# scrose/SVDSolver

Measured on NVIDIA B200. Metric: bidiag_reduction_gflops, higher is better.
Workload: dtype f64,f32

## Files before the change

svdsolver_b200/csrc/capi.cu:

```cuda
#include <algorithm>
#include <new>
#include "common.cuh"

using namespace svdb200;

namespace svdb200 {
template <typename T, bool kTrans> int launch_panel_public(Ctx* c, T* a, size_t lda, int m, int b, T* V, T* V2, cudaStream_t stream);
namespace {

__device__ __forceinline__ unsigned long long splitmix64(unsigned long long x) {
    x += 0x9E3779B97F4A7C15ull;
    x = (x ^ (x >> 30)) * 0xBF58476D1CE4E5B9ull;
    x = (x ^ (x >> 27)) * 0x94D049BB133111EBull;
    return x ^ (x >> 31);
}
template <typename T>
__global__ void fill_uniform_kernel(T* __restrict__ a, size_t count, unsigned long long seed, double lo, double hi) {
    size_t i = (size_t)blockIdx.x * blockDim.x + threadIdx.x;
    size_t stride = (size_t)gridDim.x * blockDim.x;
    const double span = __dsub_rn(hi, lo);
    for (; i < count; i += stride) {
        double u = __dmul_rn((double)(splitmix64(seed + i) >> 11), 1.0 / 9007199254740992.0);
        a[i] = (T)__dadd_rn(lo, __dmul_rn(span, u));
    }
// ... 235 lines not shown
        Ctx* s = c->pool[i % K];
        inherit_settings(c, s);
        T* ai = a + i * n * n;
        T* d = reinterpret_cast<T*>(s->d);
        T* e = reinterpret_cast<T*>(s->e);
        const long long before = s->launches;
        s->overlap_safe = (concurrent && K > 1) ? 1 : 0;
        const int st1 = stage1_panel_order<T>(s, ai, n, band);
        s->overlap_safe = 0;
        if (st1 != 0) { c->last_error = s->last_error; return st1; }
        SVDB_TRY(stage2_chase<T>(s, ai, n, band, d, e));
        SVDB_TRY(bidiag_qr<T>(s, d, e, n, sigma + i * n));
        c->launches += s->launches - before;
    }
    for (int i = 0; i < K; ++i) {
        SVDB_CHECK(c, cudaEventRecord(c->pool[i]->lev[0], c->pool[i]->stream));
        SVDB_CHECK(c, cudaStreamWaitEvent(c->stream, c->pool[i]->lev[0], 0));
    }
    return 0;
}
template <typename T>
int batched_chain(Ctx* c, T* a, size_t count, size_t n, size_t band, int what, T* d, T* e, T* sigma) {
    if (count == 0) return 0;
    if (!(n <= 1024 && band <= 64 && c->cluster_ok >= 8 && n >= 2)) return SVDB200_E_CAPACITY;
    return batched_small<T>(c, a, count, n, band, sigma, what, d, e);
}
template int batched_chain<float>(Ctx*, float*, size_t, size_t, size_t, int, float*, float*, float*);
template int batched_chain<double>(Ctx*, double*, size_t, size_t, size_t, int, double*, double*, double*);
template int batched_svdvals<float>(Ctx*, float*, size_t, size_t, size_t, float*);
template int batched_svdvals<double>(Ctx*, double*, size_t, size_t, size_t, double*);

constexpr size_t kOverlapMaxN = 4096;

static void release_s2(Ctx* c) {
    for (int l = 0; l < Ctx::kLanes; ++l) {
        if (c->s1ctx[l]) { svdb200_destroy(reinterpret_cast<svdb200_handle>(c->s1ctx[l])); c->s1ctx[l] = nullptr; }
        if (l > 0 && c->s2_prog[l]) cudaFree(c->s2_prog[l]);
        c->s2_prog[l] = nullptr;
        if (c->s2_stream[l]) { cudaStreamDestroy(c->s2_stream[l]); c->s2_stream[l] = nullptr; }
    }
    for (auto& e : c->s2ev) if (e) { cudaEventDestroy(e); e = nullptr; }
    c->s2_ready = 0;
}

static int ensure_s2_impl(Ctx* c) {
    for (int l = 0; l < Ctx::kLanes; ++l) {
        SVDB_CHECK(c, cudaStreamCreateWithFlags(&c->s2_stream[l], cudaStreamNonBlocking));
        if (l == 0) c->s2_prog[l] = c->prog;
        else SVDB_CHECK(c, cudaMalloc(&c->s2_prog[l], sizeof(int) * (c->max_n + 8)));
        svdb200_handle h = nullptr;
        int st = svdb200_create(&h, c->device, c->max_n, c->band, c->dtype);
        if (st != 0) return st;
        c->s1ctx[l] = reinterpret_cast<Ctx*>(h);
    }
    for (auto& e : c->s2ev) SVDB_CHECK(c, cudaEventCreateWithFlags(&e, cudaEventDisableTiming));
    return 0;
}

static int ensure_s2(Ctx* c) {
    if (c->s2_ready) return 0;
    const int st = ensure_s2_impl(c);
    if (st != 0) { release_s2(c); return st; }
    c->s2_ready = 1;
    return 0;
}

static int lanes_for(Ctx* c, size_t n, size_t band) {
    const size_t ctas = n / band / 2 + 2;
    const size_t cap = (size_t)c->num_sms - 8;
    return ((size_t)Ctx::kLanes * ctas <= cap) ? Ctx::kLanes : 1;
}

template <typename T>
static int run_stage2_on_lane(Ctx* c, int lane, T* a, size_t n, size_t band, T* d, T* e) {
    cudaStream_t s0 = c->stream;
    int* p0 = c->prog;
    c->stream = c->s2_stream[lane];
    c->prog = c->s2_prog[lane];
    const int st = stage2_chase<T>(c, a, n, band, d, e);
    c->stream = s0;
    c->prog = p0;
    return st;
}

static int drain_into(Ctx* c, cudaStream_t into) {
    for (int l = 0; l < Ctx::kLanes; ++l) {
        SVDB_CHECK(c, cudaEventRecord(c->s2ev[4 + l], c->s2_stream[l]));
        SVDB_CHECK(c, cudaStreamWaitEvent(into, c->s2ev[4 + l], 0));
        SVDB_CHECK(c, cudaEventRecord(c->s1ctx[l]->lev[0], c->s1ctx[l]->stream));
        SVDB_CHECK(c, cudaStreamWaitEvent(into, c->s1ctx[l]->lev[0], 0));
    }
    return 0;
}

template <typename T>
static int pipeline_one(Ctx* c, size_t i, T* a_dev, const T* a_host, size_t n, size_t band, int order, T* d, T* e, cudaStream_t* lane_out,
                        int k) {
    const bool overlap = order == SVDB200_ORDER_PANEL && n <= kOverlapMaxN && !c->profile;
    const int nl = overlap ? lanes_for(c, n, band) : 1;
    if (!overlap || nl == 1) {
        SVDB_TRY(drain_into(c, c->stream));
        if (a_host) SVDB_CHECK(c, cudaMemcpyAsync(a_dev, a_host, sizeof(T) * n * n, cudaMemcpyHostToDevice, c->stream));
        SVDB_TRY(order == SVDB200_ORDER_PANEL ? stage1_panel_order<T>(c, a_dev, n, band) : stage1_tile_order<T>(c, a_dev, n, band));
        if (i < c->band_capture.size() && c->band_capture[i])
            SVDB_CHECK(c, cudaMemcpyAsync(c->band_capture[i], a_dev, sizeof(T) * n * n, cudaMemcpyDeviceToDevice, c->stream));
        SVDB_TRY(stage2_chase<T>(c, a_dev, n, band, d, e));
        SVDB_CHECK(c, cudaEventRecord(c->s2ev[1], c->stream));
        for (int l = 0; l < Ctx::kLanes; ++l) {
            SVDB_CHECK(c, cudaStreamWaitEvent(c->s2_stream[l], c->s2ev[1], 0));
            SVDB_CHECK(c, cudaStreamWaitEvent(c->s1ctx[l]->stream, c->s2ev[1], 0));
        }
        *lane_out = c->stream;
        return 0;
    }
    Ctx* s = c->s1ctx[k];
    inherit_settings(c, s);
    if (a_host) SVDB_CHECK(c, cudaMemcpyAsync(a_dev, a_host, sizeof(T) * n * n, cudaMemcpyHostToDevice, s->stream));
    s->overlap_safe = 1;
    int st = stage1_panel_order<T>(s, a_dev, n, band);
    s->overlap_safe = 0;
    c->launches += s->launches; s->launches = 0;
    if (st != 0) { c->last_error = s->last_error; return st; }
    if (i < c->band_capture.size() && c->band_capture[i])
        SVDB_CHECK(c, cudaMemcpyAsync(c->band_capture[i], a_dev, sizeof(T) * n * n, cudaMemcpyDeviceToDevice, s->stream));
    SVDB_CHECK(c, cudaEventRecord(s->lev[0], s->stream));
    SVDB_CHECK(c, cudaStreamWaitEvent(c->s2_stream[k], s->lev[0], 0));
    SVDB_TRY(run_stage2_on_lane<T>(c, k, a_dev, n, band, d, e));
    *lane_out = c->s2_stream[k];
    return 0;
}

struct ListPlan { std::vector<size_t> order; std::vector<int> chain; };
static ListPlan plan_list(int lanes, size_t count, const size_t* n) {
    ListPlan pl;
    const int L = lanes < 1 ? 1 : lanes;
    pl.order.reserve(count); pl.chain.reserve(count);
    if (L == 1 || count <= (size_t)L) {
        for (size_t i = 0; i < count; ++i) { pl.order.push_back(i); pl.chain.push_back((int)(i % (size_t)L)); }
        return pl;
    }
    std::vector<size_t> idx(count);
    for (size_t i = 0; i < count; ++i) idx[i] = i;
    std::stable_sort(idx.begin(), idx.end(), [&](size_t x, size_t y) { return n[x] > n[y]; });
    std::vector<std::vector<size_t>> items(L);
    std::vector<size_t> load(L, 0);
    for (size_t i : idx) {
        int best = 0;
        for (int l = 1; l < L; ++l) if (load[l] < load[best]) best = l;
        items[best].push_back(i);
        load[best] += n[i];
    }
    for (auto& v : items) std::stable_sort(v.begin(), v.end(), [&](size_t x, size_t y) { return n[x] != n[y] ? n[x] < n[y] : x < y; });
    for (size_t t = 0; pl.order.size() < count; ++t)
        for (int l = 0; l < L; ++l)
            if (t < items[l].size()) { pl.order.push_back(items[l][t]); pl.chain.push_back(l); }
    return pl;
}

template <typename T>
int bidiagonalize_many_dev(Ctx* c, size_t count, T* const* a, const size_t* n, size_t band, int order, T* const* d, T* const* e) {
    if (count == 0) return 0;
    SVDB_TRY(ensure_s2(c));
    cudaStream_t s0 = c->stream;
    SVDB_CHECK(c, cudaEventRecord(c->s2ev[0], s0));
    for (int l = 0; l < Ctx::kLanes; ++l) {
        SVDB_CHECK(c, cudaStreamWaitEvent(c->s2_stream[l], c->s2ev[0], 0));
        SVDB_CHECK(c, cudaStreamWaitEvent(c->s1ctx[l]->stream, c->s2ev[0], 0));
    }
    const ListPlan pl = plan_list(Ctx::kLanes, count, n);
    for (size_t j = 0; j < count; ++j) {
        const size_t i = pl.order[j];
        cudaStream_t lane;
        SVDB_TRY(pipeline_one<T>(c, i, a[i], (const T*)nullptr, n[i], band, order, d ? d[i] : nullptr, e ? e[i] : nullptr, &lane, pl.chain[j]));
    }
    const int sj = drain_into(c, s0);
    c->band_capture.clear();
    return sj;
}
template int bidiagonalize_many_dev<float>(Ctx*, size_t, float* const*, const size_t*, size_t, int, float* const*, float* const*);
template int bidiagonalize_many_dev<double>(Ctx*, size_t, double* const*, const size_t*, size_t, int, double* const*, double* const*);

static bool is_pageable(const void* p) {
    if (!p) return false;
    cudaPointerAttributes at{};
    if (cudaPointerGetAttributes(&at, p) != cudaSuccess) { cudaGetLastError(); return true; }
    return at.type == cudaMemoryTypeUnregistered;
}

template <typename T>
int bidiagonalize_many_host(Ctx* c, size_t count, T* const* a, const size_t* n, size_t band, int order, T* const* d, T* const* e) {
    if (count == 0) return 0;
    SVDB_TRY(ensure_s2(c));
    constexpr int NB = 2 * Ctx::kLanes;
    if (!c->a_dev) SVDB_CHECK(c, cudaMalloc(&c->a_dev, c->esz * c->max_n * c->max_n));
    c->a_stage[0] = c->a_dev;
    for (int k = 1; k < NB; ++k)
        if (!c->a_stage[k]) SVDB_CHECK(c, cudaMalloc(&c->a_stage[k], c->esz * c->max_n * c->max_n));
    if (!c->de2) SVDB_CHECK(c, cudaMalloc(&c->de2, c->esz * 2 * NB * (c->max_n + 8)));
    cudaStream_t s0 = c->stream;
    SVDB_CHECK(c, cudaEventRecord(c->s2ev[0], s0));
    for (int l = 0; l < Ctx::kLanes; ++l) {
        SVDB_CHECK(c, cudaStreamWaitEvent(c->s2_stream[l], c->s2ev[0], 0));
        SVDB_CHECK(c, cudaStreamWaitEvent(c->s1ctx[l]->stream, c->s2ev[0], 0));
    }
    struct EvSet {
        cudaEvent_t ev[NB] = {};
        ~EvSet() { for (auto& x : ev) if (x) cudaEventDestroy(x); }
    } evs;
    cudaEvent_t* ev_free = evs.ev;
    for (auto& ev : evs.ev) SVDB_CHECK(c, cudaEventCreateWithFlags(&ev, cudaEventDisableTiming));
    struct Result { T *a, *d, *e; size_t n; cudaStream_t lane; bool live; } res[NB] = {};
    auto copy_back = [&](int k) -> int {
        Result& r = res[k];
        if (!r.live) return 0;
        r.live = false;
        T* buf = reinterpret_cast<T*>(c->a_stage[k]);
        T* dd = reinterpret_cast<T*>(c->de2) + (size_t)2 * k * (c->max_n + 8);
        T* ee = dd + (c->max_n + 8);
        SVDB_CHECK(c, cudaMemcpyAsync(r.a, buf, sizeof(T) * r.n * r.n, cudaMemcpyDeviceToHost, r.lane));
        if (r.d) SVDB_CHECK(c, cudaMemcpyAsync(r.d, dd, sizeof(T) * r.n, cudaMemcpyDeviceToHost, r.lane));
        if (r.e) SVDB_CHECK(c, cudaMemcpyAsync(r.e, ee, sizeof(T) * (r.n - 1), cudaMemcpyDeviceToHost, r.lane));
        SVDB_CHECK(c, cudaEventRecord(ev_free[k], r.lane));
        return 0;
    };
    int st = 0;
    const ListPlan pl = plan_list(Ctx::kLanes, count, n);
    size_t per_chain[Ctx::kLanes] = {};
    bool used[NB] = {};
    for (size_t j = 0; j < count && st == 0; ++j) {
        const size_t i = pl.order[j];
        const int ch = pl.chain[j];
        const int k = ch + Ctx::kLanes * (int)(per_chain[ch]++ % 2);
        const size_t ni = n[i];
        T* buf = reinterpret_cast<T*>(c->a_stage[k]);
        T* dd = reinterpret_cast<T*>(c->de2) + (size_t)2 * k * (c->max_n + 8);
        T* ee = dd + (c->max_n + 8);
        if ((st = copy_back(k)) != 0) break;
// ... 178 lines not shown
    SVDB_CREATE_CHECK(cudaMalloc(&c->s, es * band * band));
    SVDB_CREATE_CHECK(cudaMalloc(&c->tau, es * band));
    SVDB_CREATE_CHECK(cudaMalloc(&c->red, es * 2 * (kMaxPanelCtas + 1) * (2 * band + 8)));
    SVDB_CREATE_CHECK(cudaMemset(c->red, 0, es * 2 * (kMaxPanelCtas + 1) * (2 * band + 8)));
    SVDB_CREATE_CHECK(cudaMalloc(&c->red2, 512 * 1024));
    SVDB_CREATE_CHECK(cudaMemset(c->red2, 0, 512 * 1024));
    SVDB_CREATE_CHECK(cudaMalloc(&c->chol_ws, 1 << 20));
    SVDB_CREATE_CHECK(cudaMemset(c->chol_ws, 0, 1 << 20));
    SVDB_CREATE_CHECK(cudaMalloc(&c->bar, 64));
    SVDB_CREATE_CHECK(cudaMemset(c->bar, 0, 64));
    SVDB_CREATE_CHECK(cudaMalloc(&c->prog, sizeof(int) * (max_n + 8)));
    SVDB_CREATE_CHECK(cudaMalloc(&c->d, es * (max_n + 8)));
    SVDB_CREATE_CHECK(cudaMalloc(&c->e, es * (max_n + 8)));
    SVDB_CREATE_CHECK(cudaMalloc(&c->sigma, es * (max_n + 8)));
    SVDB_CREATE_CHECK(cudaMalloc(&c->qr_info, 64));
    SVDB_CREATE_CHECK(cudaMemset(c->qr_info, 0, 64));
    SVDB_CREATE_CHECK(cudaMalloc(&c->tileq, es * (max_n / band + 2) * 4 * band * band));
    SVDB_CREATE_CHECK(cudaMalloc(&c->tilestate, es * (4 * band * band + 64)));
#undef SVDB_CREATE_CHECK
    *out = reinterpret_cast<svdb200_handle>(c);
    return 0;
}

int svdb200_destroy(svdb200_handle h) {
    if (!h) return SVDB200_E_ARG;
    Ctx* c = reinterpret_cast<Ctx*>(h);
    cudaSetDevice(c->device);
    if (c->own_stream) cudaStreamSynchronize(c->own_stream);
    for (auto& ph : c->pool) if (ph) svdb200_destroy(reinterpret_cast<svdb200_handle>(ph));
    c->pool.clear();
    void* ptrs[] = {c->a_dev, c->v, c->v2, c->vb, c->v2b, c->w, c->wpart, c->s, c->tau, c->red, c->red2, c->chol_ws, c->bar, c->prog,
                    c->d, c->e, c->sigma, c->qr_info, c->tileq, c->tilestate, c->tcsplit, c->bis_ws, c->batch_prog, c->batch_ws, c->de2};
    for (int k = 1; k < 2 * Ctx::kLanes; ++k) if (c->a_stage[k]) cudaFree(c->a_stage[k]);
    for (int l = 0; l < Ctx::kLanes; ++l) if (c->s1ctx[l]) svdb200_destroy(reinterpret_cast<svdb200_handle>(c->s1ctx[l]));
    for (int l = 1; l < Ctx::kLanes; ++l) if (c->s2_prog[l]) cudaFree(c->s2_prog[l]);
    for (void* p : ptrs) if (p) cudaFree(p);
    for (auto& e : c->ev) if (e) cudaEventDestroy(e);
    for (auto& e : c->pev) if (e) cudaEventDestroy(e);
    for (auto& e : c->lev) if (e) cudaEventDestroy(e);
    for (auto& e : c->s2ev) if (e) cudaEventDestroy(e);
    for (auto& st2 : c->s2_stream) if (st2) cudaStreamDestroy(st2);
    if (c->aux_stream) cudaStreamDestroy(c->aux_stream);
    if (c->own_stream) cudaStreamDestroy(c->own_stream);
    delete c;
    return 0;
}

int svdb200_set_stream(svdb200_handle h, void* stream) {
    if (!h) return SVDB200_E_ARG;
    Ctx* c = reinterpret_cast<Ctx*>(h);
    c->stream = stream ? reinterpret_cast<cudaStream_t>(stream) : c->own_stream;
    return 0;
}

int svdb200_synchronize(svdb200_handle h) {
    if (!h) return SVDB200_E_ARG;
    Ctx* c = reinterpret_cast<Ctx*>(h);
    SVDB_CHECK(c, cudaStreamSynchronize(c->stream));
    return 0;
}

#define SVDB_ENTER(T)                                    \
    Ctx* c = reinterpret_cast<Ctx*>(h);                  \
    if (!c) return SVDB200_E_ARG;                        \
    if (c->dtype != dtype_of<T>()) return SVDB200_E_ARG; \
    SVDB_CHECK(c, cudaSetDevice(c->device));

#define SVDB_DEFINE_TYPED(T, S)                                                                                          \
// ... 308 lines not shown
```

svdsolver_b200/csrc/common.cuh:

```cuda
#pragma once
#include <cuda_runtime.h>
#include <cstddef>
#include <cstdint>
#include <cstdio>
#include <cstring>
#include <string>
#include <vector>
#include "../../include/svdb200.h"

namespace svdb200 {

constexpr int kMaxBand = 128;
constexpr int kMaxPanelCtas = 148;
constexpr int kLookaheadReserve = 20;

struct Settings {
    int stage2_complete = 0;
    int qr_method = 0;
    size_t qr_auto_limit = 1024;
    int use_tc05 = 1;
    long long tc05_min_elems = 8LL << 20;
    int panel_blk = 1;
    int panel_chol = 1;
    double chol_guard = 1e-3;
};

struct Ctx {
    int device = 0;
    int dtype = SVDB200_F64;
    size_t max_n = 0, band = 0, esz = 8;
    int num_sms = 148;
    cudaStream_t own_stream = nullptr, stream = nullptr;
    void* a_dev = nullptr;
    void* v = nullptr;
    void* v2 = nullptr;
    void* vb = nullptr; void* v2b = nullptr;
    cudaStream_t aux_stream = nullptr;
    cudaEvent_t lev[4] = {};
    void* w = nullptr;
    void* wpart = nullptr;
    size_t wpart_elems = 0;
    void* s = nullptr;
    void* tau = nullptr;
    unsigned panel_epoch = 0;
    void* red = nullptr;
    void* red2 = nullptr;
    unsigned int* bar = nullptr;
    int* prog = nullptr;
    void* d = nullptr; void* e = nullptr; void* sigma = nullptr;
    long long* qr_info = nullptr;
    void* tileq = nullptr;
    void* tilestate = nullptr;
    long long launches = 0;
    cudaEvent_t ev[8] = {};
    double ms_stage1 = 0, ms_stage2 = 0, ms_qr = 0, ms_h2d = 0, ms_d2h = 0;
    std::string last_error;
    int coop_supported = 0;
    int cluster_ok = 16;
    int profile = 0;
    double prof_ms[SVDB200_PROFILE_CLASSES] = {};
    double prof_work[SVDB200_PROFILE_CLASSES] = {};
    long long prof_launches[SVDB200_PROFILE_CLASSES] = {};
    cudaEvent_t pev[2] = {};
    std::vector<Ctx*> pool;
    size_t pool_n = 0, pool_band = 0;
    void* tcsplit = nullptr;
    size_t tcsplit_elems = 0;
    Settings cfg;
    static constexpr int kLanes = 2;
    cudaStream_t s2_stream[kLanes] = {};
    int* s2_prog[kLanes] = {};
    cudaEvent_t s2ev[4 + kLanes] = {};
    int onestage = 0;
    int s2_ready = 0;
    void* chol_ws = nullptr;
    const int* panel_run_if = nullptr;
    int reserve_now = 0;
    int overlap_safe = 0;
    Ctx* s1ctx[kLanes] = {};
    void* a_stage[2 * kLanes] = {};
    void* de2 = nullptr;
    void* bis_ws = nullptr;
    size_t bis_ws_elems = 0;
    std::vector<void*> band_capture;
    int* batch_prog = nullptr;
    size_t batch_prog_elems = 0;
    void* batch_ws = nullptr;
    size_t batch_ws_bytes = 0;
};

struct ProfScope {
    Ctx* c; int cls; double work;
    ProfScope(Ctx* c_, int cls_, double work_) : c(c_), cls(cls_), work(work_) {
        if (c->profile) cudaEventRecord(c->pev[0], c->stream);
    }
    ~ProfScope() {
        if (!c->profile) return;
        cudaEventRecord(c->pev[1], c->stream);
        cudaEventSynchronize(c->pev[1]);
        float ms = 0;
        cudaEventElapsedTime(&ms, c->pev[0], c->pev[1]);
        c->prof_ms[cls] += ms; c->prof_work[cls] += work; c->prof_launches[cls] += 1;
    }
};

inline int cuda_status(Ctx* c, cudaError_t e, const char* what) {
    if (e == cudaSuccess) return 0;
    if (c) {
        c->last_error = std::string(what) + ": " + cudaGetErrorString(e);
    }
    return SVDB200_CUDA_ERR + (int)e;
}
// ... 41 lines not shown
    int v;
    asm volatile("ld.acquire.gpu.global.s32 %0, [%1];" : "=r"(v) : "l"(p) : "memory");
    return v;
}
__device__ __forceinline__ void st_release(int* p, int v) {
    asm volatile("st.release.gpu.global.s32 [%0], %1;" ::"l"(p), "r"(v) : "memory");
}
__device__ __forceinline__ unsigned ld_acquire_u(const unsigned* p) {
    unsigned v;
    asm volatile("ld.acquire.gpu.global.u32 %0, [%1];" : "=r"(v) : "l"(p) : "memory");
    return v;
}

__device__ __forceinline__ void grid_barrier(unsigned* bar, unsigned nctas, unsigned& gen) {
    __syncthreads();
    if (threadIdx.x == 0) {
        __threadfence();
        unsigned target = gen + 1;
        unsigned prev = atomicAdd(&bar[0], 1u);
        if (prev == nctas * target - 1) {
            asm volatile("st.release.gpu.global.u32 [%0], %1;" ::"l"(&bar[1]), "r"(target) : "memory");
        } else {
            while (ld_acquire_u(&bar[1]) < target) { __nanosleep(20); }
        }
        __threadfence();
    }
    gen += 1;
    __syncthreads();
}

template <typename T> int stage2_chase(Ctx* c, T* a, size_t n, size_t band, T* d, T* e);
template <typename T> int extract_bidiagonal(Ctx* c, const T* a, size_t n, T* d, T* e);
template <typename T> int stage2_chase_fast(Ctx* c, T* a, size_t n, size_t band, int* prog);
template <typename T> int bidiag_qr(Ctx* c, T* d, T* e, size_t n, T* sigma);
template <typename T> int bidiag_bisect(Ctx* c, const T* d, const T* e, size_t n, T* sigma);
template <typename T> int bidiag_sqr(Ctx* c, T* d, T* e, size_t n, T* sigma);
template <typename T> int stage1_panel_order(Ctx* c, T* a, size_t n, size_t band);
template <typename T> int stage1_tile_order(Ctx* c, T* a, size_t n, size_t band);
template <typename T> int gemm_tn(Ctx* c, const T* v, const T* cm, size_t ldc, size_t mrows, size_t ncols, size_t b, T* w);
template <typename T> int gemm_nn(Ctx* c, const T* cm, size_t ldc, size_t mrows, size_t ncols, size_t b, const T* ut, T* w);
template <typename T> int rank_update(Ctx* c, T* cm, size_t ldc, size_t mrows, size_t ncols, size_t b, const T* p, const T* q, size_t ldq);
template <typename T> int rank_update_batched(Ctx* c, T* cm, size_t ldc, size_t sC, int M, int N, int K, const T* p, size_t sP, const T* q, size_t ldq, size_t sQ, int count);
template <typename T> int gemm_tn_batched(Ctx* c, const T* v, size_t sV, const T* cm, size_t ldc, size_t sC, int M, int N, int B, T* w, size_t sW, int count);
template <typename T> int gemm_nn_batched(Ctx* c, const T* cm, size_t ldc, size_t sC, int M, int N, int B, const T* ut, size_t sU, T* w, size_t sW, int count);
template <typename T, bool kTrans> int panel_batched(Ctx* c, T* a, size_t lda, size_t sA, int m, int b, T* V, T* V2, size_t sV, int count);
template <typename T> int stage2_chase_batched(Ctx* c, T* a, size_t n, size_t band, T* d, T* e, int count);
template <typename T> int bidiag_bisect_batched(Ctx* c, const T* d, const T* e, size_t n, T* sigma, int count);
template <typename T> int fill_uniform(Ctx* c, T* a, size_t count, unsigned long long seed, double lo, double hi);
template <typename T> int mse_metric(Ctx* c, const T* a, const T* b, size_t n, size_t band, T* out_host);
template <typename T> int batched_svdvals(Ctx* c, T* a, size_t count, size_t n, size_t band, T* sigma);
template <typename T> int batched_chain(Ctx* c, T* a, size_t count, size_t n, size_t band, int what, T* d, T* e, T* sigma);
int probe_peak(Ctx* c, int kind, double* tflops);
int probe_tc05_tf32(Ctx* c, double* tflops);
int panel_reg_debug_read(long long* out16);
int panel_blk_debug_read(long long* out16);
int panel_chol_debug_read(long long* out16);
int stage2_debug_read(long long* out16);
int stage2_fast_debug_read(long long* out16);
int tc05_selftest(Ctx* c, int a_mn, int b_mn, const float* a, const float* b, float* out, float* dump);

}
```

svdsolver_b200/csrc/stage2_chase.cu:

```cuda
#include <algorithm>
#include <climits>
#include "common.cuh"
#include "stage2_common.cuh"

namespace svdb200 {

namespace {

#ifndef SVDB_S2_TIMING
#define SVDB_S2_TIMING 0
#endif
__device__ long long g_s2_dbg[16];
#define S2_TICK(k)                                                          \
    do {                                                                    \
        if (SVDB_S2_TIMING && blockIdx.x == 1 && threadIdx.x == 0) {        \
            long long _t = clock64();                                       \
            g_s2_dbg[k] += _t - tick;                                       \
            tick = _t;                                                      \
        }                                                                   \
    } while (0)

using namespace s2;

template <typename T, int kMaxThreads, int kMinBlocks, int kC>
// ... 106 lines not shown
                                  }, tid);
                fr = fwd ? nr : 0;
                __syncthreads();
                if (tid == rel_tid && fwd) st_release(&prog[i], q + 1);
            }
            if (!fwd) break;
        }
        if (tid == rel_tid) st_release(&prog[i], INT_MAX);
    }
    }
}

}
int stage2_debug_read(long long* out16) {
    long long z[16] = {};
    if (cudaMemcpyFromSymbol(out16, g_s2_dbg, sizeof(z)) != cudaSuccess) return 1;
    cudaMemcpyToSymbol(g_s2_dbg, z, sizeof(z));
    return 0;
}
namespace {

template <typename T>
__global__ void extract_bidiagonal_kernel(const T* __restrict__ A, int n, T* __restrict__ d, T* __restrict__ e) {
    int i = blockIdx.x * blockDim.x + threadIdx.x;
    A += (size_t)blockIdx.y * n * n;
    if (d) d += (size_t)blockIdx.y * n;
    if (e) e += (size_t)blockIdx.y * n;
    if (i < n) {
        if (d) d[i] = A[(size_t)i * n + i];
        if (e && i + 1 < n) e[i] = A[(size_t)i * n + i + 1];
    }
}

}

template <typename T>
int stage2_chase_batched(Ctx* c, T* a, size_t n, size_t band, T* d, T* e, int count) {
    if (n < 2 || band < 1 || count < 1) return SVDB200_E_SHAPE;
    if (n > (size_t)INT_MAX / 4) return SVDB200_E_CAPACITY;
    const int cb = (int)band;
    ProfScope ps(c, 4, 4.0 * (double)band * (double)n * (double)n * sizeof(T) * count);
    size_t smem = (size_t)(2 * cb * (cb + 1) + cb * (2 * cb + 1) + cb * (cb + 1) + 8) * sizeof(T);
    int nt = stage2_threads(cb);
    if (nt > 1024) return SVDB200_E_CAPACITY;
    if (cb * cb > kNewPerThread * nt) return SVDB200_E_CAPACITY;
    if (smem > 227 * 1024) return SVDB200_E_CAPACITY;
    const bool light = count > 1;
    auto kern = nt <= 256 ? (light ? stage2_chase_kernel<T, 256, 3, 0> : stage2_chase_kernel<T, 256, 1, 0>)
                          : stage2_chase_kernel<T, 1024, 1, 0>;
    if (cb == 32) kern = light ? stage2_chase_kernel<T, 256, 3, 32> : stage2_chase_kernel<T, 256, 1, 32>;
    else if (cb == 64) kern = stage2_chase_kernel<T, 1024, 1, 64>;
    SVDB_CHECK(c, cudaFuncSetAttribute(kern, cudaFuncAttributeMaxDynamicSharedMemorySize, (int)smem));
    int per_sm = 0;
    SVDB_CHECK(c, cudaOccupancyMaxActiveBlocksPerMultiprocessor(&per_sm, kern, nt, smem));
    if (per_sm < 1) return SVDB200_E_CAPACITY;
    long long inflight = (long long)(n / band) / 2 + 2;
    if (count > 1) inflight = std::max<long long>(1, (long long)(n / band + 1) / 2);
    long long slots = (long long)per_sm * c->num_sms;
    long long G = std::min(inflight, std::min(slots, (long long)n - 1));
    if (G < 1) G = 1;
    long long groups = std::min((long long)count, slots / G);
    if (groups < 1) groups = 1;
    const long long grid = groups * G;
    int* prog = c->prog;
    if (count > 1) {
        const size_t need = (size_t)count * n;
        if (c->batch_prog_elems < need) {
// ... 48 lines not shown
```

svdsolver_b200/csrc/stage2_chase_fast.cu:

```cuda
#include <algorithm>
#include <climits>
#include "common.cuh"
#include "stage2_common.cuh"

namespace svdb200 {

namespace {
using namespace s2;

#ifndef SVDB_S2_TIMING
#define SVDB_S2_TIMING 0
#endif
__device__ long long g_s2f_dbg[16];
#define S2F_T() (SVDB_S2_TIMING ? clock64() : 0ll)
#define S2F_ADD(k, v)                                                   \
    do {                                                                \
        if (SVDB_S2_TIMING && blockIdx.x == 1) g_s2f_dbg[k] += (v);     \
    } while (0)

constexpr int kC = 32;
constexpr int kMain = 256;
constexpr int kFastThreads = kMain + 32;

__device__ __forceinline__ void bar_n_helper() { asm volatile("bar.sync 1, 160;" ::: "memory"); }

template <typename T>
__device__ __forceinline__ void helper_reflector(T xv, T* __restrict__ xst, T* __restrict__ Hn, int ldh, bool guard) {
    const int lane = threadIdx.x & 31;
    xst[lane] = xv;
    __syncwarp();
    T x[kC];
    if constexpr (sizeof(T) == 4) {
#pragma unroll
        for (int r = 0; r < kC; r += 4) {
            const float4 v = *reinterpret_cast<const float4*>(xst + r);
            x[r] = v.x; x[r + 1] = v.y; x[r + 2] = v.z; x[r + 3] = v.w;
        }
    } else {
#pragma unroll
        for (int r = 0; r < kC; r += 2) {
            const double2 v = *reinterpret_cast<const double2*>(xst + r);
            x[r] = v.x; x[r + 1] = v.y;
        }
    }
    T acc = (T)0;
#pragma unroll
    for (int r = 0; r < kC; ++r) acc = RN<T>::add(acc, RN<T>::mul(x[r], x[r]));
    T alpha, tau;
    if (guard && acc == (T)0) { alpha = (T)0; tau = (T)0; }
    else householder_scalars<T>(x[0], RN<T>::sqrt(acc), alpha, tau);
    const T mtau = -tau;
    const T wl = (lane == 0) ? (T)1 : RN<T>::mul(xv, alpha);
#pragma unroll
    for (int i = 0; i < kC; ++i) {
        const T wi = (i == 0) ? (T)1 : RN<T>::mul(x[i], alpha);
        T h = RN<T>::mul(RN<T>::add((T)0, RN<T>::mul(wi, wl)), mtau);
        if (i == lane) h = RN<T>::add((T)1, h);
        Hn[i * ldh + lane] = h;
    }
    __syncwarp();
}

template <typename T>
__global__ void __launch_bounds__(kFastThreads, 1) stage2_fast_kernel(T* __restrict__ A, int n, int* __restrict__ prog, int complete) {
    extern __shared__ __align__(16) unsigned char smem_raw[];
    constexpr int c = kC, w = c + 1;
    constexpr int ldr = c + 1, ldl = 2 * c + 1, ldh = c + 1;
    T* WR = reinterpret_cast<T*>(smem_raw);
    T* WL = WR + 2 * c * ldr;
    T* Hb0 = WL + c * ldl;
    T* Hb1 = Hb0 + c * ldh;
    T* sc = Hb1 + c * ldh;
    T* xst = sc + 8;
    const int tid = threadIdx.x;
    const bool is_main = tid < kMain, is_helper = !is_main;
    const bool f_warp = tid < kMain / 2, n_warp = is_main && !f_warp;
    const size_t N = (size_t)n;
    const int tx = tid % c, ty = tid / c;
    constexpr int tys = kMain / c;
    const int ht = tid - kMain / 2;
    const int G = gridDim.x;
    const int rel_tid = 32;
    T* Hc = Hb0;
    T* Hn = Hb1;
    for (int i = blockIdx.x; i < n - 1; i += G) {
        int seen = 0;
        const int top_j2 = min(i + 2 * w - 1, n);
        const int npairs = complete ? (n - i - 1 + c - 1) / c : 1 + (n - top_j2) / c + 1;
        int fr = 0;
        bool hready = false;
        for (int p = 0; p < npairs; ++p) {
            const int r0 = (p == 0) ? i : min(i + 1 + (p - 1) * c, n);
            const int r1 = min(i + 1 + p * c, n), r2 = min(i + 1 + (p + 1) * c, n), c3 = min(i + 1 + (p + 2) * c, n);
            if (r2 <= r1) break;
            {
                const int q = 2 * p;
                const long long t_op0 = S2F_T();
                if (i > 0 && tid == 0) seen = wait_progress(&prog[i - 1], q + 4, seen);
                const long long t_polled = S2F_T();
                __syncthreads();
                const long long t_start = S2F_T();
                const int nc = r2 - r1, nr = r2 - r0, have = fr;
                const bool interior = (have == c) && (nr == 2 * c) && (nc == c);
                if (interior) {
                    if (tid == 0) { S2F_ADD(0, t_polled - t_op0); S2F_ADD(9, t_start - t_polled); S2F_ADD(7, 1); if (!hready) S2F_ADD(10, 1); }
                    T nv[8];
                    if (n_warp) {
#pragma unroll
                        for (int u = 0; u < 8; ++u) nv[u] = ld_cg(&A[(size_t)(r1 + (ht >> 5) + 4 * u) * N + (r1 + (ht & 31))]);
                    }
                    if (!hready) {
                        if (tid == 0) reflector_scalars<T>(WR, 1, c, sc, complete != 0);
                        __syncthreads();
                        if (is_main) build_h<T>(WR, 1, c, sc, Hc, ldh, tx, ty, tys);
                        __syncthreads();
                    }
                    const long long t_h = S2F_T();
                    long long t_done = 0;
// ... 40 lines not shown
                                WR[(e / nc) * ldr + e % nc] = ld_cg(&A[(size_t)(r0 + e / nc) * N + (r1 + e % nc)]);
                        __syncthreads();
                    } else if (is_main) {
#pragma unroll
                        for (int u = 0; u < kNewPerThread; ++u) {
                            int r = ty + u * tys;
                            if (r < nr - have && tx < nc) nv[u] = ld_cg(&A[(size_t)(r0 + have + r) * N + (r1 + tx)]);
                        }
                    }
                    if (!hready && tid == 0) reflector_scalars<T>(WR, 1, nc, sc, complete != 0);
                    __syncthreads();
                    if (is_main) {
                        if (!hready) build_h<T>(WR, 1, nc, sc, Hc, ldh, tx, ty, tys);
                        if (have != 0) {
#pragma unroll
                            for (int u = 0; u < kNewPerThread; ++u) {
                                int r = ty + u * tys;
                                if (r < nr - have && tx < nc) WR[(have + r) * ldr + tx] = nv[u];
                            }
                        }
                    }
                    __syncthreads();
                    const int keep = r1 - r0;
                    if (is_main)
                        window_product<T, kC>(WR, ldr, Hc, ldh, nr, nc, nc, (c + 1) / 2, (c + 1) / 2,
                                              [&](int r, int cc, T v) {
                                                  if (r < keep) st_cg(&A[(size_t)(r0 + r) * N + (r1 + cc)], v);
                                                  else WL[(r - keep) * ldl + cc] = v;
                                              }, tid);
                    __syncthreads();
                    hready = false;
                }
                if (tid == rel_tid) st_release(&prog[i], q + 1);
            }
            const int nn = c3 - r2;
            const bool fwd = (p + 1 < npairs) && nn > 0;
            {
                const int q = 2 * p + 1;
                if (i > 0 && tid == 0) seen = wait_progress(&prog[i - 1], q + 4, seen);
                __syncthreads();
                const int nr = r2 - r1, fc = r2 - r1, nc = fc + nn;
                const bool interior = (nr == c) && (nn == c) && fwd;
                if (interior) {
                    T nv[8];
                    if (n_warp) {
#pragma unroll
                        for (int u = 0; u < 8; ++u) nv[u] = ld_cg(&A[(size_t)(r1 + (ht >> 5) + 4 * u) * N + (r2 + (ht & 31))]);
                    }
                    if (!hready) {
                        if (tid == 0) reflector_scalars<T>(WL, ldl, c, sc, complete != 0);
                        __syncthreads();
                        if (is_main) build_h<T>(WL, ldl, c, sc, Hc, ldh, tx, ty, tys);
                        __syncthreads();
                    }
                    if (f_warp) {
                        window_product<T, kC>(Hc, ldh, WL, ldl, c, c, c, 16, 8,
                                              [&](int r, int cc, T v) { st_cg(&A[(size_t)(r1 + r) * N + (r1 + cc)], v); }, tid);
                    } else if (n_warp) {
#pragma unroll
                        for (int u = 0; u < 8; ++u) WL[((ht >> 5) + 4 * u) * ldl + c + (ht & 31)] = nv[u];
                        bar_n_helper();
                        window_product<T, kC>(Hc, ldh, WL + c, ldl, c, c, c, 16, 8,
                                              [&](int r, int cc, T v) { WR[r * ldr + cc] = v; }, ht);
                    } else {
                        bar_n_helper();
                        const int lane = tid & 31;
                        T xo[kC], yo[kC];
#pragma unroll
                        for (int k = 0; k < c; ++k) { xo[k] = Hc[k]; yo[k] = WL[k * ldl + c + lane]; }
                        T acc = (T)0;
#pragma unroll
                        for (int k = 0; k < c; ++k) acc = RN<T>::add(acc, RN<T>::mul(xo[k], yo[k]));
// ... 4 lines not shown
                    { T* t = Hc; Hc = Hn; Hn = t; }
                    hready = true;
                } else {
                    T nv[kNewPerThread];
                    if (is_main) {
#pragma unroll
                        for (int u = 0; u < kNewPerThread; ++u) {
                            int r = ty + u * tys;
                            if (r < nr && tx < nn) nv[u] = ld_cg(&A[(size_t)(r1 + r) * N + (r2 + tx)]);
                        }
                    }
                    if (!hready && tid == 0) reflector_scalars<T>(WL, ldl, nr, sc, complete != 0);
                    __syncthreads();
                    if (is_main) {
                        if (!hready) build_h<T>(WL, ldl, nr, sc, Hc, ldh, tx, ty, tys);
#pragma unroll
                        for (int u = 0; u < kNewPerThread; ++u) {
                            int r = ty + u * tys;
                            if (r < nr && tx < nn) WL[r * ldl + fc + tx] = nv[u];
                        }
                    }
                    __syncthreads();
                    if (is_main)
                        window_product<T, kC>(Hc, ldh, WL, ldl, nr, nc, nr, c, (c + 3) / 4,
                                              [&](int r, int cc, T v) {
                                                  if (cc < fc || !fwd) st_cg(&A[(size_t)(r1 + r) * N + (r1 + cc)], v);
                                                  else WR[r * ldr + (cc - fc)] = v;
                                              }, tid);
                    fr = fwd ? nr : 0;
                    __syncthreads();
                    hready = false;
                }
                if (tid == rel_tid && fwd) st_release(&prog[i], q + 1);
            }
            if (!fwd) break;
        }
        if (tid == rel_tid) st_release(&prog[i], INT_MAX);
    }
}

}

int stage2_fast_debug_read(long long* out16) {
    long long z[16] = {};
    if (cudaMemcpyFromSymbol(out16, g_s2f_dbg, sizeof(z)) != cudaSuccess) return 1;
    cudaMemcpyToSymbol(g_s2f_dbg, z, sizeof(z));
    return 0;
}

template <typename T>
int stage2_chase_fast(Ctx* c, T* a, size_t n, size_t band, int* prog) {
    if (band != (size_t)kC || n < 2 * band + 2) return 1;
    const size_t smem = (size_t)(2 * kC * (kC + 1) + kC * (2 * kC + 1) + 2 * kC * (kC + 1) + 8 + kC + 8) * sizeof(T);
    auto kern = stage2_fast_kernel<T>;
    SVDB_CHECK(c, cudaFuncSetAttribute(kern, cudaFuncAttributeMaxDynamicSharedMemorySize, (int)smem));
    int per_sm = 0;
    SVDB_CHECK(c, cudaOccupancyMaxActiveBlocksPerMultiprocessor(&per_sm, kern, kFastThreads, smem));
    if (per_sm < 1) return 1;
    long long inflight = (long long)(n / band) / 2 + 2;
    long long G = std::min(inflight, std::min((long long)per_sm * c->num_sms, (long long)n - 1));
    if (G < 1) G = 1;
    int ni = (int)n, complete = c->cfg.stage2_complete;
    void* args[] = {&a, &ni, &prog, &complete};
    SVDB_CHECK(c, cudaLaunchCooperativeKernel((void*)kern, dim3((unsigned)G), dim3(kFastThreads), args, smem, c->stream));
    c->launches++;
    return 0;
}
template int stage2_chase_fast<float>(Ctx*, float*, size_t, size_t, int*);
template int stage2_chase_fast<double>(Ctx*, double*, size_t, size_t, int*);

}
```

Baseline: 2993.

## Add pooled stage-2 bulge-chase kernel with work-stealing across matrix lists

```diff
diff --git a/svdsolver_b200/csrc/capi.cu b/svdsolver_b200/csrc/capi.cu
--- a/svdsolver_b200/csrc/capi.cu
+++ b/svdsolver_b200/csrc/capi.cu
@@ -291,13 +291,17 @@
 
 constexpr size_t kOverlapMaxN = 4096;
 
+static_assert(Ctx::kChains >= Ctx::kLanes, "the lane path runs stage 1 of lane k on sub-handle k");
+
 static void release_s2(Ctx* c) {
     for (int l = 0; l < Ctx::kLanes; ++l) {
-        if (c->s1ctx[l]) { svdb200_destroy(reinterpret_cast<svdb200_handle>(c->s1ctx[l])); c->s1ctx[l] = nullptr; }
         if (l > 0 && c->s2_prog[l]) cudaFree(c->s2_prog[l]);
         c->s2_prog[l] = nullptr;
         if (c->s2_stream[l]) { cudaStreamDestroy(c->s2_stream[l]); c->s2_stream[l] = nullptr; }
     }
+    for (auto& h : c->s1ctx) if (h) { svdb200_destroy(reinterpret_cast<svdb200_handle>(h)); h = nullptr; }
+    for (auto& st : c->pool_stream) if (st) { cudaStreamDestroy(st); st = nullptr; }
+    if (c->pool_copied) { cudaEventDestroy(c->pool_copied); c->pool_copied = nullptr; }
     for (auto& e : c->s2ev) if (e) { cudaEventDestroy(e); e = nullptr; }
     c->s2_ready = 0;
 }
@@ -307,11 +311,15 @@
         SVDB_CHECK(c, cudaStreamCreateWithFlags(&c->s2_stream[l], cudaStreamNonBlocking));
         if (l == 0) c->s2_prog[l] = c->prog;
         else SVDB_CHECK(c, cudaMalloc(&c->s2_prog[l], sizeof(int) * (c->max_n + 8)));
+    }
+    for (auto& sub : c->s1ctx) {
         svdb200_handle h = nullptr;
         int st = svdb200_create(&h, c->device, c->max_n, c->band, c->dtype);
         if (st != 0) return st;
-        c->s1ctx[l] = reinterpret_cast<Ctx*>(h);
-    }
+        sub = reinterpret_cast<Ctx*>(h);
+    }
+    for (auto& st : c->pool_stream) SVDB_CHECK(c, cudaStreamCreateWithFlags(&st, cudaStreamNonBlocking));
+    SVDB_CHECK(c, cudaEventCreateWithFlags(&c->pool_copied, cudaEventDisableTiming));
     for (auto& e : c->s2ev) SVDB_CHECK(c, cudaEventCreateWithFlags(&e, cudaEventDisableTiming));
     return 0;
 }
@@ -342,12 +350,20 @@
     return st;
 }
 
+static int fan_out(Ctx* c, cudaEvent_t ev) {
+    for (int l = 0; l < Ctx::kLanes; ++l) SVDB_CHECK(c, cudaStreamWaitEvent(c->s2_stream[l], ev, 0));
+    for (Ctx* s : c->s1ctx) SVDB_CHECK(c, cudaStreamWaitEvent(s->stream, ev, 0));
+    return 0;
+}
+
 static int drain_into(Ctx* c, cudaStream_t into) {
     for (int l = 0; l < Ctx::kLanes; ++l) {
         SVDB_CHECK(c, cudaEventRecord(c->s2ev[4 + l], c->s2_stream[l]));
         SVDB_CHECK(c, cudaStreamWaitEvent(into, c->s2ev[4 + l], 0));
-        SVDB_CHECK(c, cudaEventRecord(c->s1ctx[l]->lev[0], c->s1ctx[l]->stream));
-        SVDB_CHECK(c, cudaStreamWaitEvent(into, c->s1ctx[l]->lev[0], 0));
+    }
+    for (Ctx* s : c->s1ctx) {
+        SVDB_CHECK(c, cudaEventRecord(s->lev[0], s->stream));
+        SVDB_CHECK(c, cudaStreamWaitEvent(into, s->lev[0], 0));
     }
     return 0;
 }
@@ -365,10 +381,8 @@
             SVDB_CHECK(c, cudaMemcpyAsync(c->band_capture[i], a_dev, sizeof(T) * n * n, cudaMemcpyDeviceToDevice, c->stream));
         SVDB_TRY(stage2_chase<T>(c, a_dev, n, band, d, e));
         SVDB_CHECK(c, cudaEventRecord(c->s2ev[1], c->stream));
-        for (int l = 0; l < Ctx::kLanes; ++l) {
-            SVDB_CHECK(c, cudaStreamWaitEvent(c->s2_stream[l], c->s2ev[1], 0));
-            SVDB_CHECK(c, cudaStreamWaitEvent(c->s1ctx[l]->stream, c->s2ev[1], 0));
-        }
+        for (int l = 0; l < Ctx::kLanes; ++l) SVDB_CHECK(c, cudaStreamWaitEvent(c->s2_stream[l], c->s2ev[1], 0));
+        for (Ctx* s : c->s1ctx) SVDB_CHECK(c, cudaStreamWaitEvent(s->stream, c->s2ev[1], 0));
         *lane_out = c->stream;
         return 0;
     }
@@ -416,16 +430,99 @@
     return pl;
 }
 
+static bool pool_applies(const Ctx* c, size_t count, const size_t* n, size_t band, int order) {
+    if (order != SVDB200_ORDER_PANEL || band != 32 || c->profile) return false;
+    for (size_t i = 0; i < count; ++i)
+        if (n[i] > kOverlapMaxN || n[i] < 2 * band + 2) return false;
+    return true;
+}
+
+static int ensure_pool_buffers(Ctx* c, size_t count, size_t prog_elems) {
+    if (c->pool_tab_cap < count) {
+        SVDB_CHECK(c, cudaEventSynchronize(c->pool_copied));
+        if (c->pool_tab) cudaFree(c->pool_tab);
+        if (c->pool_tab_host) cudaFreeHost(c->pool_tab_host);
+        c->pool_tab = c->pool_tab_host = nullptr; c->pool_tab_cap = 0;
+        const size_t bytes = sizeof(PoolHdr) + sizeof(PoolMat) * count;
+        SVDB_CHECK(c, cudaMalloc(&c->pool_tab, bytes));
+        SVDB_CHECK(c, cudaMallocHost(&c->pool_tab_host, bytes));
+        c->pool_tab_cap = count;
+    }
+    if (c->pool_prog_elems < prog_elems) {
+        if (c->pool_prog) cudaFree(c->pool_prog);
+        c->pool_prog = nullptr; c->pool_prog_elems = 0;
+        SVDB_CHECK(c, cudaMalloc(&c->pool_prog, sizeof(int) * prog_elems));
+        c->pool_prog_elems = prog_elems;
+    }
+    return 0;
+}
+
+template <typename T>
+static int bidiagonalize_many_pool(Ctx* c, size_t count, T* const* a, const size_t* n, size_t band, T* const* d, T* const* e) {
+    const ListPlan pl = plan_list(Ctx::kChains, count, n);
+    size_t prog_elems = 0, max_n = 0;
+    for (size_t i = 0; i < count; ++i) { prog_elems += n[i]; max_n = std::max(max_n, n[i]); }
+    SVDB_TRY(ensure_pool_buffers(c, count, prog_elems));
+    cudaStream_t s0 = c->stream;
+    SVDB_CHECK(c, cudaEventSynchronize(c->pool_copied));
+    PoolHdr* hh = reinterpret_cast<PoolHdr*>(c->pool_tab_host);
+    PoolMat* hm = reinterpret_cast<PoolMat*>(hh + 1);
+    *hh = PoolHdr{};
+    for (size_t j = 0, off = 0; j < count; ++j) {
+        const size_t i = pl.order[j];
+        hm[j] = PoolMat{a[i], d ? d[i] : nullptr, e ? e[i] : nullptr, (int)n[i], (int)off, stage2_pool_cap(n[i]), 0, 0, 0};
+        off += n[i];
+    }
+    const size_t tab_bytes = sizeof(PoolHdr) + sizeof(PoolMat) * count;
+    SVDB_CHECK(c, cudaMemcpyAsync(c->pool_tab, c->pool_tab_host, tab_bytes, cudaMemcpyHostToDevice, s0));
+    SVDB_CHECK(c, cudaEventRecord(c->pool_copied, s0));
+    SVDB_CHECK(c, cudaMemsetAsync(c->pool_prog, 0, sizeof(int) * prog_elems, s0));
+    SVDB_CHECK(c, cudaEventRecord(c->s2ev[0], s0));
+    SVDB_TRY(fan_out(c, c->s2ev[0]));
+    for (cudaStream_t ps : c->pool_stream) SVDB_CHECK(c, cudaStreamWaitEvent(ps, c->s2ev[0], 0));
+    PoolHdr* hdr = reinterpret_cast<PoolHdr*>(c->pool_tab);
+    const int max_running = std::max(1, c->num_sms - Ctx::kPoolReserve);
+    bool issued[Ctx::kChains] = {};
+    for (size_t j = 0; j < count; ++j) {
+        const size_t i = pl.order[j];
+        const int k = pl.chain[j];
+        Ctx* s = c->s1ctx[k];
+        inherit_settings(c, s);
+        s->overlap_safe = 1;
+        const int st = stage1_panel_order<T>(s, a[i], n[i], band);
+        s->overlap_safe = 0;
+        c->launches += s->launches; s->launches = 0;
+        if (st != 0) { c->last_error = s->last_error; return st; }
+        if (i < c->band_capture.size() && c->band_capture[i])
+            SVDB_CHECK(c, cudaMemcpyAsync(c->band_capture[i], a[i], sizeof(T) * n[i] * n[i], cudaMemcpyDeviceToDevice, s->stream));
+        SVDB_CHECK(c, cudaEventRecord(s->lev[0], s->stream));
+        issued[k] = true;
+        cudaStream_t ps = c->pool_stream[j % Ctx::kPoolStreams];
+        for (int l = 0; l < Ctx::kChains; ++l)
+            if (issued[l]) SVDB_CHECK(c, cudaStreamWaitEvent(ps, c->s1ctx[l]->lev[0], 0));
+        SVDB_TRY(stage2_pool_launch<T>(c, ps, hdr, c->pool_prog, (int)j + 1, hm[j].cap, max_running));
+    }
+    SVDB_TRY(drain_into(c, s0));
+    for (cudaStream_t ps : c->pool_stream) {
+        SVDB_CHECK(c, cudaEventRecord(c->s2ev[1], ps));
+        SVDB_CHECK(c, cudaStreamWaitEvent(s0, c->s2ev[1], 0));
+    }
+    if (d || e) SVDB_TRY(extract_bidiagonal_list<T>(c, reinterpret_cast<const PoolMat*>(hdr + 1), (int)count, max_n, s0));
+    return 0;
+}
+
 template <typename T>
 int bidiagonalize_many_dev(Ctx* c, size_t count, T* const* a, const size_t* n, size_t band, int order, T* const* d, T* const* e) {
     if (count == 0) return 0;
     SVDB_TRY(ensure_s2(c));
+    if (pool_applies(c, count, n, band, order)) {
+        const int st = bidiagonalize_many_pool<T>(c, count, a, n, band, d, e);
+        c->band_capture.clear();
+        return st;
+    }
     cudaStream_t s0 = c->stream;
     SVDB_CHECK(c, cudaEventRecord(c->s2ev[0], s0));
-    for (int l = 0; l < Ctx::kLanes; ++l) {
-        SVDB_CHECK(c, cudaStreamWaitEvent(c->s2_stream[l], c->s2ev[0], 0));
-        SVDB_CHECK(c, cudaStreamWaitEvent(c->s1ctx[l]->stream, c->s2ev[0], 0));
-    }
+    SVDB_TRY(fan_out(c, c->s2ev[0]));
     const ListPlan pl = plan_list(Ctx::kLanes, count, n);
     for (size_t j = 0; j < count; ++j) {
         const size_t i = pl.order[j];
@@ -458,10 +555,7 @@
     if (!c->de2) SVDB_CHECK(c, cudaMalloc(&c->de2, c->esz * 2 * NB * (c->max_n + 8)));
     cudaStream_t s0 = c->stream;
     SVDB_CHECK(c, cudaEventRecord(c->s2ev[0], s0));
-    for (int l = 0; l < Ctx::kLanes; ++l) {
-        SVDB_CHECK(c, cudaStreamWaitEvent(c->s2_stream[l], c->s2ev[0], 0));
-        SVDB_CHECK(c, cudaStreamWaitEvent(c->s1ctx[l]->stream, c->s2ev[0], 0));
-    }
+    SVDB_TRY(fan_out(c, c->s2ev[0]));
     struct EvSet {
         cudaEvent_t ev[NB] = {};
         ~EvSet() { for (auto& x : ev) if (x) cudaEventDestroy(x); }
@@ -706,8 +800,13 @@
     void* ptrs[] = {c->a_dev, c->v, c->v2, c->vb, c->v2b, c->w, c->wpart, c->s, c->tau, c->red, c->red2, c->chol_ws, c->bar, c->prog,
                     c->d, c->e, c->sigma, c->qr_info, c->tileq, c->tilestate, c->tcsplit, c->bis_ws, c->batch_prog, c->batch_ws, c->de2};
     for (int k = 1; k < 2 * Ctx::kLanes; ++k) if (c->a_stage[k]) cudaFree(c->a_stage[k]);
-    for (int l = 0; l < Ctx::kLanes; ++l) if (c->s1ctx[l]) svdb200_destroy(reinterpret_cast<svdb200_handle>(c->s1ctx[l]));
+    for (Ctx* s : c->s1ctx) if (s) svdb200_destroy(reinterpret_cast<svdb200_handle>(s));
     for (int l = 1; l < Ctx::kLanes; ++l) if (c->s2_prog[l]) cudaFree(c->s2_prog[l]);
+    if (c->pool_tab) cudaFree(c->pool_tab);
+    if (c->pool_tab_host) cudaFreeHost(c->pool_tab_host);
+    if (c->pool_prog) cudaFree(c->pool_prog);
+    for (auto& st : c->pool_stream) if (st) cudaStreamDestroy(st);
+    if (c->pool_copied) cudaEventDestroy(c->pool_copied);
     for (void* p : ptrs) if (p) cudaFree(p);
     for (auto& e : c->ev) if (e) cudaEventDestroy(e);
     for (auto& e : c->pev) if (e) cudaEventDestroy(e);
diff --git a/svdsolver_b200/csrc/common.cuh b/svdsolver_b200/csrc/common.cuh
--- a/svdsolver_b200/csrc/common.cuh
+++ b/svdsolver_b200/csrc/common.cuh
@@ -23,6 +23,23 @@
     int panel_blk = 1;
     int panel_chol = 1;
     double chol_guard = 1e-3;
+};
+
+struct PoolHdr {
+    int running;
+    int ready;
+    int pad[2];
+};
+struct PoolMat {
+    void* a;
+    void* d;
+    void* e;
+    int n;
+    int prog_off;
+    int cap;
+    int next;
+    int done;
+    int pad;
 };
 
 struct Ctx {
@@ -68,6 +85,9 @@
     size_t tcsplit_elems = 0;
     Settings cfg;
     static constexpr int kLanes = 2;
+    static constexpr int kChains = 2;
+    static constexpr int kPoolStreams = 16;
+    static constexpr int kPoolReserve = 8;
     cudaStream_t s2_stream[kLanes] = {};
     int* s2_prog[kLanes] = {};
     cudaEvent_t s2ev[4 + kLanes] = {};
@@ -77,7 +97,14 @@
     const int* panel_run_if = nullptr;
     int reserve_now = 0;
     int overlap_safe = 0;
-    Ctx* s1ctx[kLanes] = {};
+    Ctx* s1ctx[kChains] = {};
+    cudaStream_t pool_stream[kPoolStreams] = {};
+    void* pool_tab = nullptr;
+    void* pool_tab_host = nullptr;
+    size_t pool_tab_cap = 0;
+    int* pool_prog = nullptr;
+    size_t pool_prog_elems = 0;
+    cudaEvent_t pool_copied = nullptr;
     void* a_stage[2 * kLanes] = {};
     void* de2 = nullptr;
     void* bis_ws = nullptr;
@@ -185,6 +212,9 @@
 template <typename T> int stage2_chase(Ctx* c, T* a, size_t n, size_t band, T* d, T* e);
 template <typename T> int extract_bidiagonal(Ctx* c, const T* a, size_t n, T* d, T* e);
 template <typename T> int stage2_chase_fast(Ctx* c, T* a, size_t n, size_t band, int* prog);
+int stage2_pool_cap(size_t n);
+template <typename T> int stage2_pool_launch(Ctx* c, cudaStream_t s, PoolHdr* hdr, int* prog, int ready, int grid, int max_running);
+template <typename T> int extract_bidiagonal_list(Ctx* c, const PoolMat* mats, int count, size_t max_n, cudaStream_t s);
 template <typename T> int bidiag_qr(Ctx* c, T* d, T* e, size_t n, T* sigma);
 template <typename T> int bidiag_bisect(Ctx* c, const T* d, const T* e, size_t n, T* sigma);
 template <typename T> int bidiag_sqr(Ctx* c, T* d, T* e, size_t n, T* sigma);
diff --git a/svdsolver_b200/csrc/stage2_chase.cu b/svdsolver_b200/csrc/stage2_chase.cu
--- a/svdsolver_b200/csrc/stage2_chase.cu
+++ b/svdsolver_b200/csrc/stage2_chase.cu
@@ -162,7 +162,30 @@
     }
 }
 
-}
+template <typename T>
+__global__ void extract_bidiagonal_list_kernel(const PoolMat* __restrict__ mats) {
+    const PoolMat& m = mats[blockIdx.y];
+    const int i = blockIdx.x * blockDim.x + threadIdx.x, n = m.n;
+    const T* A = reinterpret_cast<const T*>(m.a);
+    T* d = reinterpret_cast<T*>(m.d);
+    T* e = reinterpret_cast<T*>(m.e);
+    if (i < n) {
+        if (d) d[i] = A[(size_t)i * n + i];
+        if (e && i + 1 < n) e[i] = A[(size_t)i * n + i + 1];
+    }
+}
+
+}
+
+template <typename T>
+int extract_bidiagonal_list(Ctx* c, const PoolMat* mats, int count, size_t max_n, cudaStream_t s) {
+    extract_bidiagonal_list_kernel<T><<<dim3((unsigned)((max_n + 255) / 256), (unsigned)count), 256, 0, s>>>(mats);
+    SVDB_CHECK(c, cudaGetLastError());
+    c->launches++;
+    return 0;
+}
+template int extract_bidiagonal_list<float>(Ctx*, const PoolMat*, int, size_t, cudaStream_t);
+template int extract_bidiagonal_list<double>(Ctx*, const PoolMat*, int, size_t, cudaStream_t);
 
 template <typename T>
 int stage2_chase_batched(Ctx* c, T* a, size_t n, size_t band, T* d, T* e, int count) {
diff --git a/svdsolver_b200/csrc/stage2_chase_fast.cu b/svdsolver_b200/csrc/stage2_chase_fast.cu
--- a/svdsolver_b200/csrc/stage2_chase_fast.cu
+++ b/svdsolver_b200/csrc/stage2_chase_fast.cu
@@ -13,6 +13,10 @@
 #endif
 __device__ long long g_s2f_dbg[16];
 #define S2F_T() (SVDB_S2_TIMING ? clock64() : 0ll)
+#define S2F_ATOMIC(k, v)                                                                                 \
+    do {                                                                                                 \
+        if (SVDB_S2_TIMING) atomicAdd(reinterpret_cast<unsigned long long*>(&g_s2f_dbg[k]), (unsigned long long)(v)); \
+    } while (0)
 #define S2F_ADD(k, v)                                                   \
     do {                                                                \
         if (SVDB_S2_TIMING && blockIdx.x == 1) g_s2f_dbg[k] += (v);     \
@@ -62,28 +66,45 @@
 }
 
 template <typename T>
-__global__ void __launch_bounds__(kFastThreads, 1) stage2_fast_kernel(T* __restrict__ A, int n, int* __restrict__ prog, int complete) {
-    extern __shared__ __align__(16) unsigned char smem_raw[];
+struct FastSmem {
+    T* WR;
+    T* WL;
+    T* Hb0;
+    T* Hb1;
+    T* sc;
+    T* xst;
+    __device__ explicit FastSmem(unsigned char* raw) {
+        constexpr int c = kC;
+        WR = reinterpret_cast<T*>(raw);
+        WL = WR + 2 * c * (c + 1);
+        Hb0 = WL + c * (2 * c + 1);
+        Hb1 = Hb0 + c * (c + 1);
+        sc = Hb1 + c * (c + 1);
+        xst = sc + 8;
+    }
+};
+template <typename T>
+constexpr size_t fast_smem_bytes() { return (size_t)(2 * kC * (kC + 1) + kC * (2 * kC + 1) + 2 * kC * (kC + 1) + 8 + kC + 8) * sizeof(T); }
+
+template <typename T>
+__device__ __forceinline__ void fast_sweep(T* __restrict__ A, int n, int* __restrict__ prog, int i, int complete, const FastSmem<T>& sm) {
     constexpr int c = kC, w = c + 1;
     constexpr int ldr = c + 1, ldl = 2 * c + 1, ldh = c + 1;
-    T* WR = reinterpret_cast<T*>(smem_raw);
-    T* WL = WR + 2 * c * ldr;
-    T* Hb0 = WL + c * ldl;
-    T* Hb1 = Hb0 + c * ldh;
-    T* sc = Hb1 + c * ldh;
-    T* xst = sc + 8;
+    T* WR = sm.WR;
+    T* WL = sm.WL;
+    T* sc = sm.sc;
+    T* xst = sm.xst;
     const int tid = threadIdx.x;
-    const bool is_main = tid < kMain, is_helper = !is_main;
+    const bool is_main = tid < kMain;
     const bool f_warp = tid < kMain / 2, n_warp = is_main && !f_warp;
     const size_t N = (size_t)n;
     const int tx = tid % c, ty = tid / c;
     constexpr int tys = kMain / c;
     const int ht = tid - kMain / 2;
-    const int G = gridDim.x;
     const int rel_tid = 32;
-    T* Hc = Hb0;
-    T* Hn = Hb1;
-    for (int i = blockIdx.x; i < n - 1; i += G) {
+    T* Hc = sm.Hb0;
+    T* Hn = sm.Hb1;
+    {
         int seen = 0;
         const int top_j2 = min(i + 2 * w - 1, n);
         const int npairs = complete ? (n - i - 1 + c - 1) / c : 1 + (n - top_j2) / c + 1;
@@ -190,12 +211,14 @@
                     hready = false;
                 }
                 if (tid == rel_tid) st_release(&prog[i], q + 1);
+                if (tid == 0) S2F_ATOMIC(15, S2F_T() - t_polled);
             }
             const int nn = c3 - r2;
             const bool fwd = (p + 1 < npairs) && nn > 0;
             {
                 const int q = 2 * p + 1;
                 if (i > 0 && tid == 0) seen = wait_progress(&prog[i - 1], q + 4, seen);
+                const long long t_polled = S2F_T();
                 __syncthreads();
                 const int nr = r2 - r1, fc = r2 - r1, nc = fc + nn;
                 const bool interior = (nr == c) && (nn == c) && fwd;
@@ -266,6 +289,7 @@
                     hready = false;
                 }
                 if (tid == rel_tid && fwd) st_release(&prog[i], q + 1);
+                if (tid == 0) S2F_ATOMIC(15, S2F_T() - t_polled);
             }
             if (!fwd) break;
         }
@@ -273,6 +297,58 @@
     }
 }
 
+template <typename T>
+__global__ void __launch_bounds__(kFastThreads, 1) stage2_fast_kernel(T* __restrict__ A, int n, int* __restrict__ prog, int complete) {
+    extern __shared__ __align__(16) unsigned char smem_raw[];
+    const FastSmem<T> sm(smem_raw);
+    for (int i = blockIdx.x; i < n - 1; i += gridDim.x) fast_sweep<T>(A, n, prog, i, complete, sm);
+}
+
+template <typename T>
+__global__ void __launch_bounds__(kFastThreads, 1) stage2_pool_kernel(PoolHdr* __restrict__ hdr, int* __restrict__ prog, int ready,
+                                                                   int max_running, int complete) {
+    extern __shared__ __align__(16) unsigned char smem_raw[];
+    __shared__ int claim[2];
+    const FastSmem<T> sm(smem_raw);
+    PoolMat* mats = reinterpret_cast<PoolMat*>(hdr + 1);
+    const long long t_life = S2F_T();
+    if (threadIdx.x == 0) {
+        int ok = atomicAdd(&hdr->running, 1) < max_running;
+        if (!ok) atomicSub(&hdr->running, 1);
+        else { __threadfence(); atomicMax(&hdr->ready, ready); }
+        claim[0] = ok;
+    }
+    __syncthreads();
+    if (!claim[0]) return;
+    for (;;) {
+        if (threadIdx.x == 0) {
+            int m = -1, i = 0;
+            const int rd = ld_acquire(&hdr->ready);
+            for (int k = 0; k < rd && m < 0; ++k) {
+                volatile PoolMat* pm = mats + k;
+                const int last = pm->n - 1, cap = pm->cap;
+                int nx = pm->next;
+                while (nx < last && nx - pm->done < cap) {
+                    const int got = atomicCAS(&mats[k].next, nx, nx + 1);
+                    if (got == nx) { m = k; i = nx; break; }
+                    nx = got;
+                }
+            }
+            claim[0] = m; claim[1] = i;
+        }
+        __syncthreads();
+        const int m = claim[0], i = claim[1];
+        if (m < 0) break;
+        const PoolMat& pm = mats[m];
+        fast_sweep<T>(reinterpret_cast<T*>(pm.a), pm.n, prog + pm.prog_off, i, complete, sm);
+        __syncthreads();
+        if (threadIdx.x == 0) atomicAdd(&mats[m].done, 1);
+    }
+    if (threadIdx.x == 0) {
+        atomicSub(&hdr->running, 1);
+        S2F_ATOMIC(14, S2F_T() - t_life);
+    }
+}
 }
 
 int stage2_fast_debug_read(long long* out16) {
@@ -285,14 +361,13 @@
 template <typename T>
 int stage2_chase_fast(Ctx* c, T* a, size_t n, size_t band, int* prog) {
     if (band != (size_t)kC || n < 2 * band + 2) return 1;
-    const size_t smem = (size_t)(2 * kC * (kC + 1) + kC * (2 * kC + 1) + 2 * kC * (kC + 1) + 8 + kC + 8) * sizeof(T);
+    const size_t smem = fast_smem_bytes<T>();
     auto kern = stage2_fast_kernel<T>;
     SVDB_CHECK(c, cudaFuncSetAttribute(kern, cudaFuncAttributeMaxDynamicSharedMemorySize, (int)smem));
     int per_sm = 0;
     SVDB_CHECK(c, cudaOccupancyMaxActiveBlocksPerMultiprocessor(&per_sm, kern, kFastThreads, smem));
     if (per_sm < 1) return 1;
-    long long inflight = (long long)(n / band) / 2 + 2;
-    long long G = std::min(inflight, std::min((long long)per_sm * c->num_sms, (long long)n - 1));
+    long long G = std::min((long long)stage2_pool_cap(n), (long long)per_sm * c->num_sms);
     if (G < 1) G = 1;
     int ni = (int)n, complete = c->cfg.stage2_complete;
     void* args[] = {&a, &ni, &prog, &complete};
@@ -303,4 +378,19 @@
 template int stage2_chase_fast<float>(Ctx*, float*, size_t, size_t, int*);
 template int stage2_chase_fast<double>(Ctx*, double*, size_t, size_t, int*);
 
-}
+int stage2_pool_cap(size_t n) { return (int)std::min<size_t>(n / kC / 2 + 2, n - 1); }
+
+template <typename T>
+int stage2_pool_launch(Ctx* c, cudaStream_t s, PoolHdr* hdr, int* prog, int ready, int grid, int max_running) {
+    const size_t smem = fast_smem_bytes<T>();
+    auto kern = stage2_pool_kernel<T>;
+    SVDB_CHECK(c, cudaFuncSetAttribute(kern, cudaFuncAttributeMaxDynamicSharedMemorySize, (int)smem));
+    kern<<<grid, kFastThreads, smem, s>>>(hdr, prog, ready, max_running, c->cfg.stage2_complete);
+    SVDB_CHECK(c, cudaGetLastError());
+    c->launches++;
+    return 0;
+}
+template int stage2_pool_launch<float>(Ctx*, cudaStream_t, PoolHdr*, int*, int, int, int);
+template int stage2_pool_launch<double>(Ctx*, cudaStream_t, PoolHdr*, int*, int, int, int);
+
+}
```

Result: slower. 2788, median of 6 (-6.8%).
